# MikeWangWZHL/VidIL

Hardware: AMD Instinct MI355X
Metric: frames/sec whole-node (BLIP caption+filt + CLIP visual-token) 224^2 8f/video (higher is better)
Workload: dtype bf16

## Files before the change

vidil_amd/csrc/gemm4w.hip:

```cpp
#include <type_traits>
#include <utility>

#include "common.h"
#include "gemm_epilogue.h"

#define VIDIL_EPI_LAZY 1
#define VIDIL_EPI_NIT TM
#define VIDIL_EPI_VIEW16 C3

namespace {

constexpr int SLOT = 16384;
template <int TM> constexpr int kBuf = (TM == 4 ? 4 : 3) * SLOT;
template <int TM> constexpr int kRing = 2 * kBuf<TM>;
template <int TM> constexpr int kLds = kRing<TM> + 4 * 8192;

template <class F, int... Is>
__device__ __forceinline__ void static_for_impl(F&& f, std::integer_sequence<int, Is...>) {
  (f(std::integral_constant<int, Is>{}), ...);
}
template <int N, class F>
__device__ __forceinline__ void static_for(F&& f) {
  static_for_impl(static_cast<F&&>(f), std::make_integer_sequence<int, N>{});
}

__device__ __forceinline__ void glds16(const void* g, char* lds) {
  __builtin_amdgcn_global_load_lds((const __attribute__((address_space(1))) void*)g,
                                   (__attribute__((address_space(3))) void*)lds, 16, 0, 0);
}

template <typename T, typename TO, int EPI, int ACT, bool FOLD, bool STATS, bool RLN, int TM = 4, bool C3 = false>
__global__ __launch_bounds__(256) void gemm4w_kernel(const vidil_gemm_args p) {
  static_assert(TM == 4 || TM == 2, "256- or 128-row output tiles");
  static_assert(!C3 || (sizeof(T) == 2 && !FOLD && !RLN && !STATS), "the in-loop compensated product: 16-bit operands, plain epilogues");
  constexpr int ESZ_OF_T = sizeof(T);
  static_assert(TM == 4 || !(FOLD || RLN), "the 128-row form is built without the row-statistics epilogues");
  constexpr int BUF = kBuf<TM>, RING_BYTES = kRing<TM>;
  constexpr int MSH = TM == 4 ? 8 : 7;
  constexpr int NPIECE = TM == 4 ? 16 : 12;
  constexpr bool ROWSTAT = FOLD || RLN;
  constexpr bool BIAS_LDS = EPI == VIDIL_EPI_F16 || EPI == VIDIL_EPI_HEADS || EPI == VIDIL_EPI_ARENA || EPI == VIDIL_EPI_F8;
  static_assert(!(FOLD && RLN), "a GEMM normalises either its A rows or its residual rows");
  static_assert(!RLN || EPI == VIDIL_EPI_F32, "the residual exists in the f32 epilogue only");
  using f16 = TO;
  using f16x4 = typename Elt<TO>::x4;
  using f16x8 = typename Elt<TO>::x8;
  using Frag = typename Mma<T>::Frag;
  constexpr int KS = Mma<T>::KS;
  constexpr int ESZ = sizeof(T);
  constexpr int KT = 128 / ESZ;
  static_assert(!FOLD || ESZ == 2, "the LayerNorm fold reads 16-bit A fragments");
  extern __shared__ __attribute__((aligned(16))) char smem[];
  const int tid = threadIdx.x;
  const int lane = tid & 63;
  const int wave = __builtin_amdgcn_readfirstlane(tid >> 6);
  const int grp = wave >> 1;
  const int wc2 = wave & 1;
  const int hi = lane >> 5, l31 = lane & 31;

  const int M = p.M, N = p.N, K = p.K;
  const int lda = p.lda > 0 ? p.lda : K;
  const int tiles_n = (N + 255) >> 8;
  const int tiles_m = (M + (1 << MSH) - 1) >> MSH;
  auto tile_of = [&](int lt, int& tm, int& tn) {
    tm = lt / tiles_n;
    tn = lt - tm * tiles_n;
  };
  int logical, remaining;
  const int tile_step = gridDim.x >= 8 ? (gridDim.x >> 3) : 1;
  {
    const int nblk = tiles_m * tiles_n;
    const int bid = blockIdx.x;
    const int xcd = bid & 7, q = nblk >> 3, r = nblk & 7, slot = bid >> 3;
    logical = (xcd < r ? xcd * (q + 1) : r * (q + 1) + (xcd - r) * q) + slot;
    remaining = (xcd < r ? q + 1 : q) - slot;
  }
  if (remaining <= 0) return;
  constexpr int KBYTES = C3 ? 64 : 128;
  const int nk = C3 ? (K / 3) / 32 : K / KT;

  int h_r0, h_c16, h_c16w;
  {
    const int r0 = tid >> 3, sl = tid & 7;
    h_r0 = r0;
    h_c16 = (sl ^ ((r0 >> 1) & 7)) * 16;
    h_c16w = h_c16;
    if constexpr (C3) {
      const int ssl = sl ^ ((r0 >> 1) & 7);
      const int plane = (K / 3) * (int)sizeof(T);
      h_c16 = (ssl & 3) * 16 + (ssl >> 2) * plane;
      h_c16w = (ssl & 3) * 16 + (ssl >> 2) * 2 * plane;
    }
  }
  const char* hbaseA = (const char*)p.A;
  const char* hbaseW = (const char*)p.W;
  int h_limA = 0, h_limW = 0;
  int h_logical = logical, h_remaining = remaining, h_kt = 0, h_buf = 0;
  bool h_live = true;
  const uint32_t pitchA = (uint32_t)lda * ESZ, pitchW = (uint32_t)K * ESZ;
  auto head_setup = [&](int lt) {
    int tile_m, tile_n;
    tile_of(lt, tile_m, tile_n);
    const int hm0 = tile_m << MSH, hn0 = tile_n << 8;
    hbaseA = (const char*)p.A + (size_t)hm0 * pitchA;
    hbaseW = (const char*)p.W + (size_t)hn0 * pitchW;
    h_limA = M - 1 - hm0;
    h_limW = N - 1 - hn0;
  };
  head_setup(logical);
  constexpr int WSLOT = TM == 4 ? 2 : 1;
  auto issue_piece = [&](int pc) {
    const int sl = pc >> 2, i = pc & 3;
    char* dst = smem + h_buf * BUF + (sl < 2 ? WSLOT + sl : sl - 2) * SLOT + i * 4096 + wave * 1024;
    asm volatile("" : "+v"(h_r0));
    const int row = h_r0 + (sl & 1) * 128 + i * 32;
#if defined(VIDIL_4W_ABLATE) && (VIDIL_4W_ABLATE & 4)
    if (p.M > 0) return;
#endif
    if (sl < 2) {
      const int rr = row < h_limW ? row : h_limW;
      glds16(hbaseW + (size_t)(h_kt * KBYTES) + ((uint32_t)rr * pitchW + (uint32_t)(C3 ? h_c16w : h_c16)), dst);
    } else {
      const int rr = row < h_limA ? row : h_limA;
      glds16(hbaseA + (size_t)(h_kt * KBYTES) + ((uint32_t)rr * pitchA + (uint32_t)h_c16), dst);
    }
  };
  auto head_advance = [&]() {
    h_buf ^= 1;
    if (h_live && ++h_kt == nk) {
      if (h_remaining > tile_step) {
        h_kt = 0;
        h_logical += tile_step;
        h_remaining -= tile_step;
        head_setup(h_logical);
      } else {
        h_kt = nk - 1;
        h_live = false;
      }
    }
  };

  f32x16 accA[TM][2], accB[TM][2];
#define ACC(i, j) ((j) < 2 ? accA[i][(j) & 1] : accB[i][(j) & 1])
  f32x4 acc16A[2 * TM][4], acc16B[2 * TM][4];
#define ACC16(mi, nj) ((nj) < 4 ? acc16A[mi][(nj) & 3] : acc16B[mi][(nj) & 3])
  float st_s[4], st_ss[4];
  f32x2 st_raw[4][4], st_sum[4];

  const int sw = (l31 >> 1) & 7;
  const int a_off = (TM == 4 ? grp * SLOT : grp * 8192) + l31 * 128;
  const int w_off = (WSLOT + wc2) * SLOT + l31 * 128;
  Frag fa[KS][TM], fw[KS][4];
  constexpr int KH = KS / 2;
  constexpr int NKS = 4 * TM;
  constexpr int NM = NKS * KS;
  constexpr int NFK = 4 + TM;
  constexpr int NFR = KH * NFK;
  constexpr int STEP = (ESZ == 2 && TM == 4) ? 2 : 1;
#ifndef VIDIL_4W_TA
#define VIDIL_4W_TA 21
#endif
  constexpr int T_A = TM == 2 ? NFR + 1 : (ESZ == 2 ? VIDIL_4W_TA : 10);
  constexpr int T_B = T_A + NPIECE * STEP;
  static_assert(T_B < NM - 2 && NFR <= T_A, "schedule");
  constexpr int NMI = 2 * TM;
  constexpr int NP = 8 * NMI;
  constexpr int NM3 = 3 * NP;
  constexpr int C3_TA = 1 + 8 + NMI;
  constexpr int C3_STEP = TM == 4 ? 6 : 2;
  constexpr int C3_TB = C3_TA + NPIECE * C3_STEP;
  static_assert(!C3 || C3_TB + 1 < 2 * NP, "C3 schedule: tile g+1 has landed before product 2 reads it");
  using Frag16 = typename Mma16<T>::Frag;
  Frag16 ga[2][NMI], gw[2][8];
  const int kq = lane >> 4, sw16 = ((lane & 15) >> 1) & 7;
  const int a_off16 = (TM == 4 ? grp * SLOT : grp * 8192) + (lane & 15) * 128;
  const int w_off16 = (WSLOT + wc2) * SLOT + (lane & 15) * 128;
  auto read_a16 = [&](const char* buf, int plane, int t) {
    if constexpr (C3) ga[plane][t] = Mma16<T>::load(buf + a_off16 + t * 2048, plane, kq, sw16);
  };
  auto read_w16 = [&](const char* buf, int plane, int t) {
    if constexpr (C3) gw[plane][t] = Mma16<T>::load(buf + w_off16 + t * 2048, plane, kq, sw16);
  };
  auto read_frag = [&](const char* buf, int ks, int r) {
#if defined(VIDIL_4W_ABLATE) && (VIDIL_4W_ABLATE & 8)
    if (p.M > 0) return;
#endif
    if (r < 4) fw[ks][r] = Mma<T>::load(buf + w_off + r * 4096, ks, hi, sw);
    else if (r - 4 < TM) fa[ks][r - 4] = Mma<T>::load(buf + a_off + (r - 4) * 4096, ks, hi, sw);
  };

#pragma unroll
  for (int pc = 0; pc < NPIECE; ++pc) issue_piece(pc);
  head_advance();
#pragma unroll
  for (int pc = 0; pc < NPIECE; ++pc) issue_piece(pc);
  head_advance();
  asm volatile("s_waitcnt vmcnt(%0)" ::"n"(NPIECE) : "memory");
  __builtin_amdgcn_s_barrier();
  int cb = 0;

  for (;;) {
    int tile_m, tile_n;
    tile_of(logical, tile_m, tile_n);
    const int m0 = tile_m << MSH, n0 = tile_n << 8;
    if constexpr (C3) {
      static_for<NMI + 8>([&](auto f_tag) {
        constexpr int f = decltype(f_tag)::value;
        if constexpr (f < NMI) read_a16(smem + cb * BUF, 0, f);
        else read_w16(smem + cb * BUF, 0, f - NMI);
      });
    } else {
      static_for<NFR>([&](auto f_tag) {
        constexpr int f = decltype(f_tag)::value;
        read_frag(smem + cb * BUF, f / NFK, f % NFK);
      });
    }
    auto iteration = [&](auto first_tag, auto last_tag) {
      constexpr bool FIRST = decltype(first_tag)::value;
      constexpr bool LAST = decltype(last_tag)::value;
      const char* const buf = smem + cb * BUF;
      const char* const nbuf = smem + (cb ^ 1) * BUF;
      static_for<NM>([&](auto n_tag) {
        constexpr int n = decltype(n_tag)::value;
        constexpr int ks = n / NKS, i = (n >> 2) % TM, j = n & 3;
        if constexpr (FIRST && ks == 0) {
          f32x16 zero = {0.f, 0.f, 0.f, 0.f, 0.f, 0.f, 0.f, 0.f, 0.f, 0.f, 0.f, 0.f, 0.f, 0.f, 0.f, 0.f};
          if constexpr (ESZ == 1) asm volatile("" : "+a"(zero));
          ACC(i, j) = Mma<T>::mma(fw[ks][j], fa[ks][i], zero);
        } else {
          ACC(i, j) = Mma<T>::mma(fw[ks][j], fa[ks][i], ACC(i, j));
        }
        if constexpr (n < NFR) read_frag(buf, KH + n / NFK, n % NFK);
        if constexpr (n == T_A) {
          __builtin_amdgcn_s_waitcnt(0xC07F);
          __builtin_amdgcn_s_barrier();
        }
        if constexpr (n > T_A && n <= T_B && (n - T_A - 1) % STEP == 0) {
          constexpr int pc = (n - T_A - 1) / STEP;
          issue_piece(pc);
          if constexpr (pc == NPIECE - 1) head_advance();
        }
        if constexpr (BIAS_LDS && LAST && n == 0) {
          if (p.bias != nullptr || FOLD || ESZ_OF_T == 1) {
            int lane_s;
            asm volatile("v_mbcnt_lo_u32_b32 %0, -1, 0\n\tv_mbcnt_hi_u32_b32 %0, -1, %0" : "=v"(lane_s));
            int col = n0 + wc2 * 128 + (lane_s & 31) * 4;
            col = col + 4 <= N ? col : N - 4;
            const float* v0 = p.bias != nullptr ? p.bias : (FOLD ? p.ln_colsum : (ESZ_OF_T == 1 ? p.w_scale : (const float*)p.W));
            const float* v1 = FOLD ? p.ln_colsum : (ESZ_OF_T == 1 ? p.w_scale : v0);
            const float* src = (lane_s < 32 ? v0 : v1) + col;
            glds16(src, smem + RING_BYTES + wave * 8192 + 4096);
          }
        }
        if constexpr (ROWSTAT && LAST && n == 0) {
          const int nparts = (FOLD ? K : N) >> 6;
          const f32x2* stats_in = (const f32x2*)p.ln_stats;
          int lane_s;
          asm volatile("v_mbcnt_lo_u32_b32 %0, -1, 0\n\tv_mbcnt_hi_u32_b32 %0, -1, %0" : "=v"(lane_s));
          const int hi = lane_s >> 5, l31 = lane_s & 31;
          const int part0 = wc2 + 2 * hi;
#pragma unroll
          for (int it = 0; it < 4; ++it) {
            int row = m0 + grp * 128 + it * 32 + l31;
            row = row < M ? row : M - 1;
#pragma unroll
            for (int q = 0; q < 4; ++q) {
              const int part = part0 + 4 * q;
              const f32x2* src = stats_in + (size_t)row * nparts + (part < nparts ? part : nparts - 1);
              asm volatile("global_load_dwordx2 %0, %1, off" : "=v"(st_raw[it][q]) : "v"(src));
            }
          }
        }
        if constexpr (n == T_B + 1) {
          asm volatile("s_waitcnt vmcnt(%0)" ::"n"(NPIECE) : "memory");
          __builtin_amdgcn_s_barrier();
        }
        if constexpr (ROWSTAT && LAST && n == T_B + 2) {
          int lane_s;
          asm volatile("v_mbcnt_lo_u32_b32 %0, -1, 0\n\tv_mbcnt_hi_u32_b32 %0, -1, %0" : "=v"(lane_s));
          const int nparts = (FOLD ? K : N) >> 6;
          const int part0 = wc2 + 2 * (lane_s >> 5);
#pragma unroll
          for (int it = 0; it < 4; ++it) {
#pragma unroll
            for (int q = 0; q < 4; ++q) {
              asm volatile("" : "+v"(st_raw[it][q]));
              if (part0 + 4 * q >= nparts) st_raw[it][q] = f32x2{0.f, 0.f};
            }
            st_sum[it] = f32x2{(st_raw[it][0][0] + st_raw[it][2][0]) + (st_raw[it][1][0] + st_raw[it][3][0]),
                               (st_raw[it][0][1] + st_raw[it][2][1]) + (st_raw[it][1][1] + st_raw[it][3][1])};
          }
        }
        if constexpr (n > T_B + 1 && !LAST) {
          constexpr int SLOTS = NM - T_B - 2;
          constexpr int PER = (NFR + SLOTS - 1) / SLOTS;
          constexpr int s = n - T_B - 2;
          static_for<PER>([&](auto q_tag) {
            constexpr int f = s * PER + decltype(q_tag)::value;
            if constexpr (f < NFR) read_frag(nbuf, f / NFK, f % NFK);
          });
        }
        __builtin_amdgcn_sched_barrier(0);
      });
      cb ^= 1;
    };
    auto iteration_c3 = [&](auto first_tag, auto last_tag) {
      constexpr bool FIRST = decltype(first_tag)::value;
      constexpr bool LAST = decltype(last_tag)::value;
      const char* const buf = smem + cb * BUF;
      const char* const nbuf = smem + (cb ^ 1) * BUF;
      static_for<NM3>([&](auto n_tag) {
        constexpr int n = decltype(n_tag)::value;
        constexpr int pr = n / NP, nj = (n / NMI) & 7, mi = n % NMI;
        constexpr int pa = pr == 2 ? 1 : 0, pw = pr == 1 ? 1 : 0;
        if constexpr (FIRST && pr == 0) Mma16<T>::mma_zero(gw[pw][nj], ga[pa][mi], ACC16(mi, nj));
        else Mma16<T>::mma(gw[pw][nj], ga[pa][mi], ACC16(mi, nj));
        if constexpr (!FIRST && n == 0) read_w16(buf, 0, 7);
        if constexpr (n >= 1 && n < 9) read_w16(buf, 1, n - 1);
        if constexpr (n >= 9 && n < 9 + NMI) read_a16(buf, 1, n - 9);
        if constexpr (n == C3_TA) {
          __builtin_amdgcn_s_waitcnt(0xC07F);
          __builtin_amdgcn_s_barrier();
        }
        if constexpr (n > C3_TA && n <= C3_TB && (n - C3_TA - 1) % C3_STEP == 0) {
          constexpr int pc = (n - C3_TA - 1) / C3_STEP;
          issue_piece(pc);
          if constexpr (pc == NPIECE - 1) head_advance();
        }
        if constexpr (BIAS_LDS && LAST && n == 0) {
          if (p.bias != nullptr) {
            int lane_s;
            asm volatile("v_mbcnt_lo_u32_b32 %0, -1, 0\n\tv_mbcnt_hi_u32_b32 %0, -1, %0" : "=v"(lane_s));
            int col = n0 + wc2 * 128 + (lane_s & 31) * 4;
            col = col + 4 <= N ? col : N - 4;
            glds16(p.bias + col, smem + RING_BYTES + wave * 8192 + 4096);
          }
        }
        if constexpr (n == C3_TB + 1) {
          asm volatile("s_waitcnt vmcnt(%0)" ::"n"(NPIECE) : "memory");
          __builtin_amdgcn_s_barrier();
        }
        if constexpr (!LAST) {
          if constexpr (n >= 2 * NP && n < 2 * NP + NMI) read_a16(nbuf, 0, n - 2 * NP);
          if constexpr (n >= 2 * NP + NMI && (n - 2 * NP) % NMI == 0) read_w16(nbuf, 0, (n - 2 * NP) / NMI - 1);
        }
        __builtin_amdgcn_sched_barrier(0);
      });
      if constexpr (LAST) mma16_settle();
      cb ^= 1;
    };
    if constexpr (C3) {
      if (nk == 1) {
        iteration_c3(std::true_type{}, std::true_type{});
      } else {
        iteration_c3(std::true_type{}, std::false_type{});
        for (int u = 2; u < nk; ++u) iteration_c3(std::false_type{}, std::false_type{});
        iteration_c3(std::false_type{}, std::true_type{});
      }
    } else if (nk == 1) {
      iteration(std::true_type{}, std::true_type{});
    } else {
      iteration(std::true_type{}, std::false_type{});
      for (int u = 2; u < nk; ++u) iteration(std::false_type{}, std::false_type{});
      iteration(std::false_type{}, std::true_type{});
    }

    int lane_e;
    asm volatile("v_mbcnt_lo_u32_b32 %0, -1, 0\n\tv_mbcnt_hi_u32_b32 %0, -1, %0" : "=v"(lane_e));
    const int lane = lane_e, hi = lane_e >> 5, l31 = lane_e & 31;
    if constexpr (ROWSTAT) {
      auto stats_blk = [&](int b) { return (f32x2*)(smem + RING_BYTES + (b >> 1) * 8192 + 4096 + 1024 + (b & 1) * 1024); };
#pragma unroll
      for (int it = 0; it < 4; ++it) stats_blk(grp * 4 + wc2 + 2 * hi)[it * 32 + l31] = st_sum[it];
      asm volatile("s_waitcnt lgkmcnt(0)" ::: "memory");
      __builtin_amdgcn_s_barrier();
      int kdiv = FOLD ? K : N;
      asm volatile("" : "+s"(kdiv));
      const float inv_k = 1.0f / (float)kdiv;
#pragma unroll
      for (int it = 0; it < 4; ++it) {
        float s = 0.f, ss = 0.f;
#pragma unroll
        for (int w = 0; w < 4; ++w) {
          const f32x2 v = stats_blk(grp * 4 + w)[it * 32 + l31];
          s += v[0];
          ss += v[1];
        }
        const float mean = s * inv_k;
        float var = ss * inv_k - mean * mean;
        var = var > 0.f ? var : 0.f;
        const float rstd = 1.0f / sqrtf(var + p.ln_eps);
        st_s[it] = rstd;
        st_ss[it] = mean * rstd;
      }
      if constexpr (RLN) {
        asm volatile("s_waitcnt lgkmcnt(0)" ::: "memory");
        __builtin_amdgcn_s_barrier();
      }
    }

    const int m_w = m0 + grp * (32 * TM);
    char* const ep = smem + RING_BYTES + wave * 8192;
#if defined(VIDIL_4W_ABLATE) && (VIDIL_4W_ABLATE & 1)
    if (p.M > 0) {
      float s = 0.f;
#pragma unroll
      for (int it = 0; it < TM; ++it)
#pragma unroll
        for (int j = 0; j < 2; ++j) s += accA[it][j][0] + accB[it][j][5];
      if (s == 123.456f) ((float*)p.out)[lane] = s;
    } else
#endif
    {
#if defined(VIDIL_4W_ABLATE) && (VIDIL_4W_ABLATE & 2)
    const int M = p.M > 0 ? 0 : 1;
#endif
#define VIDIL_EPI_BIAS_LDS 1
    {
      const int n_w = n0 + wc2 * 128;
      const char* const epb = ep + 4096;
      do {
#define acc accA
#define acc16 acc16A
#include "gemm_epilogue.inc"
#undef acc16
#undef acc
      } while (0);
    }
    {
      const int n_w = n0 + wc2 * 128 + 64;
      const char* const epb = ep + 4096 + 256;
      do {
#define acc accB
#define acc16 acc16B
#include "gemm_epilogue.inc"
#undef acc16
#undef acc
      } while (0);
    }
    }
    if (remaining <= tile_step) break;
    logical += tile_step;
    remaining -= tile_step;
  }
#undef ACC16
#undef ACC
}

template <typename T, int EPI, int ACT, bool FOLD = false, typename TO = T, bool STATS = false, bool RLN = false, int TM = 4, bool C3 = false>
int launch4w(const vidil_gemm_args& a, hipStream_t s) {
  static std::atomic<unsigned long long> attr_set{0};
  auto kern = gemm4w_kernel<T, TO, EPI, ACT, FOLD, STATS, RLN, TM, C3>;
  constexpr int LDS_BYTES = kLds<TM>;
  if (const int rc_ = vidil_lds_opt_in(attr_set, (const void*)kern, LDS_BYTES, "gemm4w")) return rc_;
  const int num_cu = vidil_cu_count() & ~7;
  const int ntiles = ((a.M + 64 * TM - 1) / (64 * TM)) * ((a.N + 255) / 256);
  const int tiles = ntiles >= num_cu ? num_cu : (ntiles >= 8 ? ((ntiles + 7) & ~7) : ntiles);
  hipLaunchKernelGGL(kern, dim3(tiles), dim3(256), LDS_BYTES, s, a);
  VIDIL_CHECK_LAUNCH("gemm4w");
  return VIDIL_OK;
}

template <typename T>
int launch4w_dispatch(const vidil_gemm_args& a, hipStream_t s) {
  if (a.ln_fold) {
    if (a.epi == VIDIL_EPI_HEADS) return launch4w<T, VIDIL_EPI_HEADS, VIDIL_ACT_NONE, true>(a, s);
    if (a.epi == VIDIL_EPI_ARENA) return launch4w<T, VIDIL_EPI_ARENA, VIDIL_ACT_NONE, true>(a, s);
    if (a.act == VIDIL_ACT_NONE) return launch4w<T, VIDIL_EPI_F16, VIDIL_ACT_NONE, true>(a, s);
    if (a.act == VIDIL_ACT_GELU_ERF) return launch4w<T, VIDIL_EPI_F16, VIDIL_ACT_GELU_ERF, true>(a, s);
    return launch4w<T, VIDIL_EPI_F16, VIDIL_ACT_QUICK_GELU, true>(a, s);
  }
  switch (a.epi) {
    case VIDIL_EPI_F16:
      if (a.act == VIDIL_ACT_NONE) return launch4w<T, VIDIL_EPI_F16, VIDIL_ACT_NONE>(a, s);
      if (a.act == VIDIL_ACT_GELU_ERF) return launch4w<T, VIDIL_EPI_F16, VIDIL_ACT_GELU_ERF>(a, s);
      return launch4w<T, VIDIL_EPI_F16, VIDIL_ACT_QUICK_GELU>(a, s);
// ... 84 lines not shown
```

vidil_amd/csrc/gemm_epilogue.inc:

```
  if (n_w >= N) break;

#ifdef VIDIL_EPI_VIEW16
  constexpr bool V16 = VIDIL_EPI_VIEW16;
  static_assert(!V16 || (!FOLD && !STATS && !RLN && ESZ == 2 && (EPI == VIDIL_EPI_F32 || EPI == VIDIL_EPI_HEADS || EPI == VIDIL_EPI_PATCH)),
                "the 16x16 accumulator view: plain f32, per-head and patch epilogues");
#else
  constexpr bool V16 = false;
#endif
  const int l15 = lane & 15, kq = lane >> 4;
  auto vw_row = [&](int g) {
    if constexpr (V16) return g * 16 + l15;
    else return l31;
  };
  auto vw_cq = [&](int g, int k) {
    if constexpr (V16) return k * 4 + kq;
    else return g * 8 + k * 2 + hi;
  };
  constexpr int NBG = V16 ? 1 : 2;

#ifdef VIDIL_EPI_NIT
  constexpr int NIT = VIDIL_EPI_NIT;
#else
  constexpr int NIT = 4;
#endif
#ifdef VIDIL_EPI_LAZY
  f32x4 q_b[2][4], q_c[2][4];
  const bool has_bias = p.bias != nullptr;
#pragma unroll
  for (int j = 0; j < 2; ++j)
#pragma unroll
    for (int rq = 0; rq < 4; ++rq) {
      q_b[j][rq] = f32x4{0.f, 0.f, 0.f, 0.f};
      q_c[j][rq] = f32x4{0.f, 0.f, 0.f, 0.f};
    }
#ifdef VIDIL_EPI_BIAS_LDS
  constexpr bool VEC_LDS = EPI == VIDIL_EPI_F16 || EPI == VIDIL_EPI_HEADS || EPI == VIDIL_EPI_ARENA || EPI == VIDIL_EPI_F8;
#else
  constexpr bool VEC_LDS = false;
#endif
  if constexpr (VEC_LDS) {
#ifdef VIDIL_EPI_BIAS_LDS
    if (has_bias) {
#pragma unroll
      for (int j = 0; j < NBG; ++j)
#pragma unroll
        for (int rq = 0; rq < 4; ++rq) q_b[j][rq] = *(const f32x4*)(epb + vw_cq(j, rq) * 4 * 4);
    }
    if constexpr (FOLD || ESZ == 1) {
#pragma unroll
      for (int j = 0; j < 2; ++j)
#pragma unroll
        for (int rq = 0; rq < 4; ++rq) q_c[j][rq] = *(const f32x4*)(epb + 512 + (j * 32 + rq * 8 + hi * 4) * 4);
    }
#endif
  } else {
    if (has_bias) {
#pragma unroll
      for (int j = 0; j < NBG; ++j)
#pragma unroll
        for (int rq = 0; rq < 4; ++rq) {
          const int col = n_w + vw_cq(j, rq) * 4;
          q_b[j][rq] = *(const f32x4*)(p.bias + (col + 4 <= N ? col : N - 4));
        }
    }
    if constexpr (FOLD || ESZ == 1) {
      const float* const cvec = FOLD ? p.ln_colsum : p.w_scale;
#pragma unroll
      for (int j = 0; j < 2; ++j)
#pragma unroll
        for (int rq = 0; rq < 4; ++rq) {
          const int col = n_w + j * 32 + rq * 8 + hi * 4;
          q_c[j][rq] = *(const f32x4*)(cvec + (col + 4 <= N ? col : N - 4));
        }
    }
  }
  auto quadrow = [&](int it, int j, f32x4 (&q4)[4]) {
    f32x2 w[8];
#pragma unroll
    for (int pi = 0; pi < 8; ++pi) {
      const int rq = pi >> 1, e = (pi & 1) * 2;
#ifdef VIDIL_EPI_VIEW16
      if constexpr (V16) w[pi] = f32x2{acc16[it * 2 + j][rq][e], acc16[it * 2 + j][rq][e + 1]};
      else
#endif
        w[pi] = f32x2{acc[it][j][rq * 4 + e], acc[it][j][rq * 4 + e + 1]};
      const f32x2 b2 = {q_b[V16 ? 0 : j][rq][e], q_b[V16 ? 0 : j][rq][e + 1]};
      if constexpr (FOLD) {
        const f32x2 c2 = {q_c[j][rq][e], q_c[j][rq][e + 1]};
        w[pi] = pk_fma(w[pi], pk_splat(st_s[it]), pk_fma(pk_splat(-st_ss[it]), c2, b2));
      } else if constexpr (ESZ == 1) {
        const f32x2 c2 = {q_c[j][rq][e], q_c[j][rq][e + 1]};
        w[pi] = pk_fma(w[pi], c2, b2);
      } else {
        w[pi] = w[pi] + b2;
      }
    }
    if constexpr (ACT == VIDIL_ACT_GELU_ERF && EPI != VIDIL_EPI_F32) {
      gelu_fast2p_n<TO, 8>(w);
    } else if constexpr (ACT != VIDIL_ACT_NONE) {
#pragma unroll
      for (int pi = 0; pi < 8; ++pi) w[pi] = ACT == VIDIL_ACT_GELU_ERF ? gelu_erf2(w[pi]) : quick_gelu2(w[pi]);
    }
#pragma unroll
    for (int rq = 0; rq < 4; ++rq) q4[rq] = f32x4{w[rq * 2][0], w[rq * 2][1], w[rq * 2 + 1][0], w[rq * 2 + 1][1]};
  };
#else
  if constexpr (FOLD) {
#pragma unroll
    for (int j = 0; j < 2; ++j)
#pragma unroll
      for (int rq = 0; rq < 4; ++rq) {
        const int col = n_w + j * 32 + rq * 8 + hi * 4;
        if (col + 4 <= N) {
          const f32x4 c4 = *(const f32x4*)(p.ln_colsum + col);
          f32x4 b4 = {0.f, 0.f, 0.f, 0.f};
          if (p.bias != nullptr) b4 = *(const f32x4*)(p.bias + col);
#pragma unroll
          for (int it = 0; it < 4; ++it)
#pragma unroll
            for (int e = 0; e < 4; ++e)
              acc[it][j][rq * 4 + e] = __builtin_fmaf(acc[it][j][rq * 4 + e], st_s[it], __builtin_fmaf(-st_ss[it], c4[e], b4[e]));
        }
      }
  } else if constexpr (ESZ == 1) {
#pragma unroll
    for (int j = 0; j < 2; ++j)
#pragma unroll
      for (int rq = 0; rq < 4; ++rq) {
        const int col = n_w + j * 32 + rq * 8 + hi * 4;
        if (col + 4 <= N) {
          const f32x4 w4 = *(const f32x4*)(p.w_scale + col);
          f32x4 b4 = {0.f, 0.f, 0.f, 0.f};
          if (p.bias != nullptr) b4 = *(const f32x4*)(p.bias + col);
#pragma unroll
          for (int it = 0; it < 4; ++it)
#pragma unroll
            for (int e = 0; e < 4; ++e) acc[it][j][rq * 4 + e] = __builtin_fmaf(acc[it][j][rq * 4 + e], w4[e], b4[e]);
        }
      }
  } else
  if (p.bias != nullptr) {
#pragma unroll
    for (int j = 0; j < 2; ++j)
#pragma unroll
      for (int rq = 0; rq < 4; ++rq) {
        const int col = n_w + j * 32 + rq * 8 + hi * 4;
        if (col + 4 <= N) {
          const f32x4 b4 = *(const f32x4*)(p.bias + col);
#pragma unroll
          for (int it = 0; it < 4; ++it)
#pragma unroll
            for (int e = 0; e < 4; ++e) acc[it][j][rq * 4 + e] += b4[e];
        }
      }
  }
  if constexpr (ACT != VIDIL_ACT_NONE) {
#pragma unroll
    for (int it = 0; it < 4; ++it)
#pragma unroll
      for (int j = 0; j < 2; ++j)
#pragma unroll
        for (int r = 0; r < 16; r += 2) {
          f32x2 v = {acc[it][j][r], acc[it][j][r + 1]};
          v = ACT == VIDIL_ACT_GELU_ERF ? (EPI == VIDIL_EPI_F32 ? gelu_erf2(v) : gelu_fast2<TO>(v)) : quick_gelu2(v);
          acc[it][j][r] = v[0];
          acc[it][j][r + 1] = v[1];
        }
  }
  auto quadrow = [&](int it, int j, f32x4 (&q4)[4]) {
#pragma unroll
    for (int rq = 0; rq < 4; ++rq) q4[rq] = f32x4{acc[it][j][rq * 4 + 0], acc[it][j][rq * 4 + 1], acc[it][j][rq * 4 + 2], acc[it][j][rq * 4 + 3]};
  };
// ... 151 lines not shown
#pragma unroll
          for (int rq = 0; rq < 4; ++rq) {
            const f32x4 q = q4[rq];
            const f32x2 q01 = f32x2{q[0], q[1]} * pk_splat(scale), q23 = f32x2{q[2], q[3]} * pk_splat(scale);
            const f16x4 v = {Elt<TO>::from_f32(q01[0]), Elt<TO>::from_f32(q01[1]), Elt<TO>::from_f32(q23[0]), Elt<TO>::from_f32(q23[1])};
            if constexpr (V16) *(f16x4*)(buf + (j * 16 + l15) * 128 + (((rq * 2 + (kq >> 1)) ^ (l15 & 7)) << 4) + (kq & 1) * 8) = v;
            else *(f16x4*)(buf + l31 * 128 + (((j * 4 + rq) ^ (l31 & 7)) << 4) + hi * 8) = v;
          }
        }
      };
      auto read_rows = [&](const char* buf, f16x8 (&v4)[4]) {
#pragma unroll
        for (int i = 0; i < 4; ++i) {
          const int row = i * 8 + (lane >> 3);
          v4[i] = *(const f16x8*)(buf + row * 128 + ((ch ^ (row & 7)) << 4));
        }
      };
      f16* hb = nullptr;
      int cap = 0, toff = 0;
      bool tiled = false;
      size_t img = 0;
      if constexpr (EPI == VIDIL_EPI_HEADS) {
        if (part == 0) { hb = (f16*)p.q; cap = p.Tq_cap; toff = 0; tiled = false; }
        else { hb = (f16*)(part == 1 ? p.k : p.vt); cap = p.Tk_cap; toff = p.t_off; tiled = p.kv_tiled != 0; }
        hb += (size_t)head * cap * 64;
        img = (size_t)p.H * cap * 64;
      }
      if constexpr (EPI == VIDIL_EPI_ARENA) {
        hb = (f16*)(part == 0 ? p.q : part == 1 ? p.k : p.vt) + head * 64;
      }
      const bool colok = n_w + ch * 8 + 8 <= N;
      __amdgpu_buffer_rsrc_t r_o16;
      uint32_t vo_o16 = 0, step_o16 = 0;
      if constexpr (EPI == VIDIL_EPI_F16) {
        const uint32_t pitch = (uint32_t)p.ldo * (uint32_t)sizeof(f16);
        const int rows_w = M - m_w < 32 * NIT ? M - m_w : 32 * NIT;
        r_o16 = uniform_rsrc((char*)p.out + ((size_t)m_w * p.ldo + n_w) * sizeof(f16), (rows_w > 0 ? (uint32_t)rows_w : 0u) * pitch);
        vo_o16 = colok ? (uint32_t)(lane >> 3) * pitch + (uint32_t)ch * 16u : 0x80000000u;
        step_o16 = 8u * pitch;
      }
      __amdgpu_buffer_rsrc_t r_hd;
      int hs_b = 0, hs_t = 0, hs_b0 = 0;
      uint32_t img_b = 0;
      if constexpr (EPI == VIDIL_EPI_HEADS) {
        const int b0 = m_w / p.T;
        hs_b0 = b0;
        r_hd = uniform_rsrc((char*)(hb + (size_t)b0 * img), 0x80000000u);
        const int m0l = m_w + (lane >> 3);
        const int bb = m0l / p.T;
        hs_t = m0l - bb * p.T;
        hs_b = bb - b0;
        img_b = (uint32_t)(img * sizeof(f16));
      }
      auto store_rows = [&](int it, f16x8 (&v4)[4]) {
        const int m_first = m_w + it * 32 + (lane >> 3);
        if constexpr (EPI == VIDIL_EPI_F16) {
#pragma unroll
          for (int i = 0; i < 4; ++i) {
            __builtin_amdgcn_raw_buffer_store_b128(__builtin_bit_cast(u32x4, v4[i]), r_o16, vo_o16, 0, 0);
            vo_o16 += step_o16;
          }
        } else if constexpr (EPI == VIDIL_EPI_HEADS) {
          auto rows4 = [&](auto tiled_tag) {
            constexpr bool TILED = decltype(tiled_tag)::value;
#pragma unroll
            for (int i = 0; i < 4; ++i) {
              const int m = m_first + i * 8;
              const uint32_t e = TILED ? (uint32_t)ktile_off(toff + hs_t, ch * 8) : (uint32_t)(toff + hs_t) * 64u + (uint32_t)ch * 8u;
              uint32_t off = (uint32_t)hs_b * img_b + e * (uint32_t)sizeof(f16);
              off = (m < M && colok) ? off : 0x80000000u;
              __builtin_amdgcn_raw_buffer_store_b128(__builtin_bit_cast(u32x4, v4[i]), r_hd, off, 0, 0);
              hs_t += 8;
              const bool wrap = hs_t >= p.T;
              hs_t = wrap ? hs_t - p.T : hs_t;
              hs_b = wrap ? hs_b + 1 : hs_b;
            }
          };
          if (tiled) {
            rows4(std::true_type{});
          } else {
            rows4(std::false_type{});
          }
        } else {
          int b = m_first / p.T, t = m_first - b * p.T;
          const size_t hd = (size_t)p.H * 64;
#pragma unroll
          for (int i = 0; i < 4; ++i) {
            const int m = m_first + i * 8;
            if (m < M && colok) {
              f16* d = hb + (part == 0 ? (size_t)m : (size_t)(p.t_off + t) * p.arena_rows + (size_t)b * p.slot_stride) * hd + ch * 8;
              *(f16x8*)d = v4[i];
            }
            t += 8;
            while (t >= p.T) { t -= p.T; ++b; }
          }
        }
      };
      f16x8 vr[4];
      compute_write(0, ep);
#pragma unroll
      for (int it = 1; it < NIT; ++it) {
        read_rows(ep, vr);
        __builtin_amdgcn_sched_barrier(0);
        compute_write(it, ep);
        __builtin_amdgcn_sched_barrier(0);
        store_rows(it - 1, vr);
        __builtin_amdgcn_sched_barrier(0);
      }
      read_rows(ep, vr);
      store_rows(NIT - 1, vr);
    }
#else
#pragma unroll
    for (int pass = 0; pass < 2; ++pass) {
#pragma unroll
      for (int i = 0; i < 2; ++i) {
        const int it = pass * 2 + i;
        const int row = i * 32 + l31;
#pragma unroll
        for (int j = 0; j < 2; ++j) {
          f32x4 q4[4];
          quadrow(it, j, q4);
#pragma unroll
          for (int rq = 0; rq < 4; ++rq) {
            const f32x4 q = q4[rq];
            const f16x4 v = {Elt<TO>::from_f32(q[0] * scale), Elt<TO>::from_f32(q[1] * scale), Elt<TO>::from_f32(q[2] * scale),
                             Elt<TO>::from_f32(q[3] * scale)};
            *(f16x4*)(ep + row * 128 + (((j * 4 + rq) ^ (row & 7)) << 4) + hi * 8) = v;
          }
        }
      }
      const int ch = lane & 7;
#pragma unroll 4
      for (int iter = 0; iter < 8; ++iter) {
        const int row = iter * 8 + (lane >> 3);
        const f16x8 v = *(const f16x8*)(ep + row * 128 + ((ch ^ (row & 7)) << 4));
        const int m = m_w + pass * 64 + row;
        const int col = n_w + ch * 8;
        if (m < M && col + 8 <= N) {
          if constexpr (EPI == VIDIL_EPI_F16) {
            *(f16x8*)((f16*)p.out + (size_t)m * p.ldo + col) = v;
          } else if constexpr (EPI == VIDIL_EPI_ARENA) {
            const int b = m / p.T, t = m - b * p.T;
            const size_t hd = (size_t)p.H * 64;
            f16* base = (f16*)(part == 0 ? p.q : part == 1 ? p.k : p.vt) + head * 64 + ch * 8;
            *(f16x8*)(base + (part == 0 ? (size_t)m : (size_t)(p.t_off + t) * p.arena_rows + (size_t)b * p.slot_stride) * hd) = v;
          } else {
            const int b = m / p.T, t = m - b * p.T;
            const size_t bh = (size_t)b * p.H + head;
            if (part == 0) {
              *(f16x8*)((f16*)p.q + (bh * p.Tq_cap + t) * 64 + ch * 8) = v;
            } else {
              f16* kv = (f16*)(part == 1 ? p.k : p.vt);
              if (p.kv_tiled) {
                *(f16x8*)(kv + bh * p.Tk_cap * 64 + ktile_off(p.t_off + t, ch * 8)) = v;
              } else {
                *(f16x8*)(kv + (bh * p.Tk_cap + p.t_off + t) * 64 + ch * 8) = v;
              }
            }
          }
        }
      }
    }
#endif
  } else {
    f32x4 rln_g = {1.f, 1.f, 1.f, 1.f}, rln_b = {0.f, 0.f, 0.f, 0.f};
    if constexpr (RLN) {
      const int col = n_w + (lane & 15) * 4;
      if (col + 4 <= N) {
        rln_g = *(const f32x4*)(p.rln_gamma + col);
        rln_b = *(const f32x4*)(p.rln_beta + col);
      }
    }
// ... 285 lines not shown
```

Before: 5163.

## Route all 16-bit GEMMs through a 16x16 MFMA pipeline with its own schedule

All 16-bit operand GEMMs, not only the C3 variant, now use the 16x16 MFMA fragment path through a new iteration_p16 loop. That loop has its own barrier and global-to-LDS piece-issue schedule, with the row-stat loads moved into it. The epilogue's 16x16 accumulator view is extended to LayerNorm-folded GEMMs: per-row stats are swizzled across lane halves and column-sum vectors are indexed in the 16x16 layout. The intent is better MFMA and LDS-read interleaving for the bf16 GEMMs. The risk is register pressure and whether the new schedule's barrier placement is correct. A small address tweak in the heads epilogue keeps the divisor in a scalar register and forces the column offset into a 64-bit vector add.

```diff
diff --git a/vidil_amd/csrc/gemm4w.hip b/vidil_amd/csrc/gemm4w.hip
--- a/vidil_amd/csrc/gemm4w.hip
+++ b/vidil_amd/csrc/gemm4w.hip
@@ -6,7 +6,7 @@
 
 #define VIDIL_EPI_LAZY 1
 #define VIDIL_EPI_NIT TM
-#define VIDIL_EPI_VIEW16 C3
+#define VIDIL_EPI_VIEW16 (ESZ_OF_T == 2)
 
 namespace {
 
@@ -145,6 +145,7 @@
   f32x4 acc16A[2 * TM][4], acc16B[2 * TM][4];
 #define ACC16(mi, nj) ((nj) < 4 ? acc16A[mi][(nj) & 3] : acc16B[mi][(nj) & 3])
   float st_s[4], st_ss[4];
+  float st16_s[4], st16_ss[4];
   f32x2 st_raw[4][4], st_sum[4];
 
   const int sw = (l31 >> 1) & 7;
@@ -156,13 +157,10 @@
   constexpr int NM = NKS * KS;
   constexpr int NFK = 4 + TM;
   constexpr int NFR = KH * NFK;
-  constexpr int STEP = (ESZ == 2 && TM == 4) ? 2 : 1;
-#ifndef VIDIL_4W_TA
-#define VIDIL_4W_TA 21
-#endif
-  constexpr int T_A = TM == 2 ? NFR + 1 : (ESZ == 2 ? VIDIL_4W_TA : 10);
+  constexpr int STEP = 1;
+  constexpr int T_A = 10;
   constexpr int T_B = T_A + NPIECE * STEP;
-  static_assert(T_B < NM - 2 && NFR <= T_A, "schedule");
+  static_assert(ESZ == 2 || (T_B < NM - 2 && NFR <= T_A), "schedule");
   constexpr int NMI = 2 * TM;
   constexpr int NP = 8 * NMI;
   constexpr int NM3 = 3 * NP;
@@ -170,16 +168,20 @@
   constexpr int C3_STEP = TM == 4 ? 6 : 2;
   constexpr int C3_TB = C3_TA + NPIECE * C3_STEP;
   static_assert(!C3 || C3_TB + 1 < 2 * NP, "C3 schedule: tile g+1 has landed before product 2 reads it");
+  constexpr int P16_TA = 8 + NMI + (TM == 4 ? 4 : 2);
+  constexpr int P16_STEP = TM == 4 ? 5 : 3;
+  constexpr int P16_TB = P16_TA + NPIECE * P16_STEP;
+  static_assert(P16_TB + 1 >= NP && P16_TB + 2 + NMI + 8 <= 2 * NP, "plain 16-bit schedule: the next tile's reads follow barrier B inside product 1");
   using Frag16 = typename Mma16<T>::Frag;
   Frag16 ga[2][NMI], gw[2][8];
   const int kq = lane >> 4, sw16 = ((lane & 15) >> 1) & 7;
   const int a_off16 = (TM == 4 ? grp * SLOT : grp * 8192) + (lane & 15) * 128;
   const int w_off16 = (WSLOT + wc2) * SLOT + (lane & 15) * 128;
   auto read_a16 = [&](const char* buf, int plane, int t) {
-    if constexpr (C3) ga[plane][t] = Mma16<T>::load(buf + a_off16 + t * 2048, plane, kq, sw16);
+    if constexpr (ESZ == 2) ga[plane][t] = Mma16<T>::load(buf + a_off16 + t * 2048, plane, kq, sw16);
   };
   auto read_w16 = [&](const char* buf, int plane, int t) {
-    if constexpr (C3) gw[plane][t] = Mma16<T>::load(buf + w_off16 + t * 2048, plane, kq, sw16);
+    if constexpr (ESZ == 2) gw[plane][t] = Mma16<T>::load(buf + w_off16 + t * 2048, plane, kq, sw16);
   };
   auto read_frag = [&](const char* buf, int ks, int r) {
 #if defined(VIDIL_4W_ABLATE) && (VIDIL_4W_ABLATE & 8)
@@ -203,7 +205,7 @@
     int tile_m, tile_n;
     tile_of(logical, tile_m, tile_n);
     const int m0 = tile_m << MSH, n0 = tile_n << 8;
-    if constexpr (C3) {
+    if constexpr (ESZ == 2) {
       static_for<NMI + 8>([&](auto f_tag) {
         constexpr int f = decltype(f_tag)::value;
         if constexpr (f < NMI) read_a16(smem + cb * BUF, 0, f);
@@ -252,44 +254,9 @@
             glds16(src, smem + RING_BYTES + wave * 8192 + 4096);
           }
         }
-        if constexpr (ROWSTAT && LAST && n == 0) {
-          const int nparts = (FOLD ? K : N) >> 6;
-          const f32x2* stats_in = (const f32x2*)p.ln_stats;
-          int lane_s;
-          asm volatile("v_mbcnt_lo_u32_b32 %0, -1, 0\n\tv_mbcnt_hi_u32_b32 %0, -1, %0" : "=v"(lane_s));
-          const int hi = lane_s >> 5, l31 = lane_s & 31;
-          const int part0 = wc2 + 2 * hi;
-#pragma unroll
-          for (int it = 0; it < 4; ++it) {
-            int row = m0 + grp * 128 + it * 32 + l31;
-            row = row < M ? row : M - 1;
-#pragma unroll
-            for (int q = 0; q < 4; ++q) {
-              const int part = part0 + 4 * q;
-              const f32x2* src = stats_in + (size_t)row * nparts + (part < nparts ? part : nparts - 1);
-              asm volatile("global_load_dwordx2 %0, %1, off" : "=v"(st_raw[it][q]) : "v"(src));
-            }
-          }
-        }
         if constexpr (n == T_B + 1) {
           asm volatile("s_waitcnt vmcnt(%0)" ::"n"(NPIECE) : "memory");
           __builtin_amdgcn_s_barrier();
-        }
-        if constexpr (ROWSTAT && LAST && n == T_B + 2) {
-          int lane_s;
-          asm volatile("v_mbcnt_lo_u32_b32 %0, -1, 0\n\tv_mbcnt_hi_u32_b32 %0, -1, %0" : "=v"(lane_s));
-          const int nparts = (FOLD ? K : N) >> 6;
-          const int part0 = wc2 + 2 * (lane_s >> 5);
-#pragma unroll
-          for (int it = 0; it < 4; ++it) {
-#pragma unroll
-            for (int q = 0; q < 4; ++q) {
-              asm volatile("" : "+v"(st_raw[it][q]));
-              if (part0 + 4 * q >= nparts) st_raw[it][q] = f32x2{0.f, 0.f};
-            }
-            st_sum[it] = f32x2{(st_raw[it][0][0] + st_raw[it][2][0]) + (st_raw[it][1][0] + st_raw[it][3][0]),
-                               (st_raw[it][0][1] + st_raw[it][2][1]) + (st_raw[it][1][1] + st_raw[it][3][1])};
-          }
         }
         if constexpr (n > T_B + 1 && !LAST) {
           constexpr int SLOTS = NM - T_B - 2;
@@ -302,6 +269,88 @@
         }
         __builtin_amdgcn_sched_barrier(0);
       });
+      cb ^= 1;
+    };
+    auto iteration_p16 = [&](auto first_tag, auto last_tag) {
+      constexpr bool FIRST = decltype(first_tag)::value;
+      constexpr bool LAST = decltype(last_tag)::value;
+      const char* const buf = smem + cb * BUF;
+      const char* const nbuf = smem + (cb ^ 1) * BUF;
+      static_for<2 * NP>([&](auto n_tag) {
+        constexpr int n = decltype(n_tag)::value;
+        constexpr int pl = n / NP, nj = (n / NMI) & 7, mi = n % NMI;
+        if constexpr (FIRST && pl == 0) Mma16<T>::mma_zero(gw[0][nj], ga[0][mi], ACC16(mi, nj));
+        else Mma16<T>::mma(gw[pl][nj], ga[pl][mi], ACC16(mi, nj));
+        if constexpr (n < 8) read_w16(buf, 1, n);
+        if constexpr (n >= 8 && n < 8 + NMI) read_a16(buf, 1, n - 8);
+        if constexpr (n == P16_TA) {
+          __builtin_amdgcn_s_waitcnt(0xC07F);
+          __builtin_amdgcn_s_barrier();
+        }
+        if constexpr (n > P16_TA && n <= P16_TB && (n - P16_TA - 1) % P16_STEP == 0) {
+          constexpr int pc = (n - P16_TA - 1) / P16_STEP;
+          issue_piece(pc);
+          if constexpr (pc == NPIECE - 1) head_advance();
+        }
+        if constexpr (BIAS_LDS && LAST && n == 0) {
+          if (p.bias != nullptr || FOLD) {
+            int lane_s;
+            asm volatile("v_mbcnt_lo_u32_b32 %0, -1, 0\n\tv_mbcnt_hi_u32_b32 %0, -1, %0" : "=v"(lane_s));
+            int col = n0 + wc2 * 128 + (lane_s & 31) * 4;
+            col = col + 4 <= N ? col : N - 4;
+            const float* v0 = p.bias != nullptr ? p.bias : p.ln_colsum;
+            const float* v1 = FOLD ? p.ln_colsum : v0;
+            const float* src = (lane_s < 32 ? v0 : v1) + col;
+            glds16(src, smem + RING_BYTES + wave * 8192 + 4096);
+          }
+        }
+        if constexpr (ROWSTAT && LAST && n == 0) {
+          const int nparts = (FOLD ? K : N) >> 6;
+          const f32x2* stats_in = (const f32x2*)p.ln_stats;
+          int lane_s;
+          asm volatile("v_mbcnt_lo_u32_b32 %0, -1, 0\n\tv_mbcnt_hi_u32_b32 %0, -1, %0" : "=v"(lane_s));
+          const int hi = lane_s >> 5, l31 = lane_s & 31;
+          const int part0 = wc2 + 2 * hi;
+#pragma unroll
+          for (int it = 0; it < 4; ++it) {
+            int row = m0 + grp * 128 + it * 32 + l31;
+            row = row < M ? row : M - 1;
+#pragma unroll
+            for (int q = 0; q < 4; ++q) {
+              const int part = part0 + 4 * q;
+              const f32x2* src = stats_in + (size_t)row * nparts + (part < nparts ? part : nparts - 1);
+              asm volatile("global_load_dwordx2 %0, %1, off" : "=v"(st_raw[it][q]) : "v"(src));
+            }
+          }
+        }
+        if constexpr (n == P16_TB + 1) {
+          asm volatile("s_waitcnt vmcnt(%0)" ::"n"(NPIECE) : "memory");
+          __builtin_amdgcn_s_barrier();
+        }
+        if constexpr (ROWSTAT && LAST && n == P16_TB + 2) {
+          int lane_s;
+          asm volatile("v_mbcnt_lo_u32_b32 %0, -1, 0\n\tv_mbcnt_hi_u32_b32 %0, -1, %0" : "=v"(lane_s));
+          const int nparts = (FOLD ? K : N) >> 6;
+          const int part0 = wc2 + 2 * (lane_s >> 5);
+#pragma unroll
+          for (int it = 0; it < 4; ++it) {
+#pragma unroll
+            for (int q = 0; q < 4; ++q) {
+              asm volatile("" : "+v"(st_raw[it][q]));
+              if (part0 + 4 * q >= nparts) st_raw[it][q] = f32x2{0.f, 0.f};
+            }
+            st_sum[it] = f32x2{(st_raw[it][0][0] + st_raw[it][2][0]) + (st_raw[it][1][0] + st_raw[it][3][0]),
+                               (st_raw[it][0][1] + st_raw[it][2][1]) + (st_raw[it][1][1] + st_raw[it][3][1])};
+          }
+        }
+        if constexpr (n > P16_TB + 1 && !LAST) {
+          constexpr int s = n - P16_TB - 2;
+          if constexpr (s < NMI) read_a16(nbuf, 0, s);
+          else if constexpr (s < NMI + 8) read_w16(nbuf, 0, s - NMI);
+        }
+        __builtin_amdgcn_sched_barrier(0);
+      });
+      if constexpr (LAST) mma16_settle();
       cb ^= 1;
     };
     auto iteration_c3 = [&](auto first_tag, auto last_tag) {
@@ -357,6 +406,14 @@
         for (int u = 2; u < nk; ++u) iteration_c3(std::false_type{}, std::false_type{});
         iteration_c3(std::false_type{}, std::true_type{});
       }
+    } else if constexpr (ESZ == 2) {
+      if (nk == 1) {
+        iteration_p16(std::true_type{}, std::true_type{});
+      } else {
+        iteration_p16(std::true_type{}, std::false_type{});
+        for (int u = 2; u < nk; ++u) iteration_p16(std::false_type{}, std::false_type{});
+        iteration_p16(std::false_type{}, std::true_type{});
+      }
     } else if (nk == 1) {
       iteration(std::true_type{}, std::true_type{});
     } else {
@@ -392,6 +449,13 @@
         const float rstd = 1.0f / sqrtf(var + p.ln_eps);
         st_s[it] = rstd;
         st_ss[it] = mean * rstd;
+      }
+      if constexpr (FOLD) {
+#pragma unroll
+        for (int it = 0; it < 4; ++it) {
+          st16_s[it] = __builtin_bit_cast(float, __builtin_amdgcn_ds_swizzle(__builtin_bit_cast(int, st_s[it]), 0x401F));
+          st16_ss[it] = __builtin_bit_cast(float, __builtin_amdgcn_ds_swizzle(__builtin_bit_cast(int, st_ss[it]), 0x401F));
+        }
       }
       if constexpr (RLN) {
         asm volatile("s_waitcnt lgkmcnt(0)" ::: "memory");
diff --git a/vidil_amd/csrc/gemm_epilogue.inc b/vidil_amd/csrc/gemm_epilogue.inc
--- a/vidil_amd/csrc/gemm_epilogue.inc
+++ b/vidil_amd/csrc/gemm_epilogue.inc
@@ -2,8 +2,7 @@
 
 #ifdef VIDIL_EPI_VIEW16
   constexpr bool V16 = VIDIL_EPI_VIEW16;
-  static_assert(!V16 || (!FOLD && !STATS && !RLN && ESZ == 2 && (EPI == VIDIL_EPI_F32 || EPI == VIDIL_EPI_HEADS || EPI == VIDIL_EPI_PATCH)),
-                "the 16x16 accumulator view: plain f32, per-head and patch epilogues");
+  static_assert(!V16 || ESZ == 2, "the 16x16 accumulator view: 16-bit operands");
 #else
   constexpr bool V16 = false;
 #endif
@@ -16,6 +15,9 @@
     if constexpr (V16) return k * 4 + kq;
     else return g * 8 + k * 2 + hi;
   };
+#ifdef VIDIL_EPI_VIEW16
+  const bool own_row[2] = {(kq & 1) == 0, (kq & 1) == 1};
+#endif
   constexpr int NBG = V16 ? 1 : 2;
 
 #ifdef VIDIL_EPI_NIT
@@ -48,9 +50,9 @@
     }
     if constexpr (FOLD || ESZ == 1) {
 #pragma unroll
-      for (int j = 0; j < 2; ++j)
-#pragma unroll
-        for (int rq = 0; rq < 4; ++rq) q_c[j][rq] = *(const f32x4*)(epb + 512 + (j * 32 + rq * 8 + hi * 4) * 4);
+      for (int j = 0; j < NBG; ++j)
+#pragma unroll
+        for (int rq = 0; rq < 4; ++rq) q_c[j][rq] = *(const f32x4*)(epb + 512 + vw_cq(j, rq) * 4 * 4);
     }
 #endif
   } else {
@@ -66,10 +68,10 @@
     if constexpr (FOLD || ESZ == 1) {
       const float* const cvec = FOLD ? p.ln_colsum : p.w_scale;
 #pragma unroll
-      for (int j = 0; j < 2; ++j)
+      for (int j = 0; j < NBG; ++j)
 #pragma unroll
         for (int rq = 0; rq < 4; ++rq) {
-          const int col = n_w + j * 32 + rq * 8 + hi * 4;
+          const int col = n_w + vw_cq(j, rq) * 4;
           q_c[j][rq] = *(const f32x4*)(cvec + (col + 4 <= N ? col : N - 4));
         }
     }
@@ -86,8 +88,12 @@
         w[pi] = f32x2{acc[it][j][rq * 4 + e], acc[it][j][rq * 4 + e + 1]};
       const f32x2 b2 = {q_b[V16 ? 0 : j][rq][e], q_b[V16 ? 0 : j][rq][e + 1]};
       if constexpr (FOLD) {
-        const f32x2 c2 = {q_c[j][rq][e], q_c[j][rq][e + 1]};
-        w[pi] = pk_fma(w[pi], pk_splat(st_s[it]), pk_fma(pk_splat(-st_ss[it]), c2, b2));
+        const f32x2 c2 = {q_c[V16 ? 0 : j][rq][e], q_c[V16 ? 0 : j][rq][e + 1]};
+#ifdef VIDIL_EPI_VIEW16
+        if constexpr (V16) w[pi] = pk_fma(w[pi], pk_splat(own_row[j] ? st_s[it] : st16_s[it]), pk_fma(pk_splat(-(own_row[j] ? st_ss[it] : st16_ss[it])), c2, b2));
+        else
+#endif
+          w[pi] = pk_fma(w[pi], pk_splat(st_s[it]), pk_fma(pk_splat(-st_ss[it]), c2, b2));
       } else if constexpr (ESZ == 1) {
         const f32x2 c2 = {q_c[j][rq][e], q_c[j][rq][e + 1]};
         w[pi] = pk_fma(w[pi], c2, b2);
@@ -405,13 +411,18 @@
             rows4(std::false_type{});
           }
         } else {
-          int b = m_first / p.T, t = m_first - b * p.T;
+          int tdiv = p.T;
+          asm volatile("" : "+s"(tdiv));
+          int b = m_first / tdiv, t = m_first - b * tdiv;
           const size_t hd = (size_t)p.H * 64;
+          uint32_t coff_hi;
+          asm volatile("v_mov_b32 %0, 0" : "=v"(coff_hi));
+          const size_t coff = ((size_t)coff_hi << 32) | (uint32_t)(ch * 8);
 #pragma unroll
           for (int i = 0; i < 4; ++i) {
             const int m = m_first + i * 8;
             if (m < M && colok) {
-              f16* d = hb + (part == 0 ? (size_t)m : (size_t)(p.t_off + t) * p.arena_rows + (size_t)b * p.slot_stride) * hd + ch * 8;
+              f16* d = hb + (part == 0 ? (size_t)m : (size_t)(p.t_off + t) * p.arena_rows + (size_t)b * p.slot_stride) * hd + coff;
               *(f16x8*)d = v4[i];
             }
             t += 8;
```

Result: faster. 5290, median of 6 (+2.5%).
